# micropilot/myosuite-mjx

Hardware: AMD Instinct MI355X
Metric: env-steps/s (whole node) myoHandPoseRandom-v0 batch 4096 (higher is better)
Workload: dtype f32

## Files before the change

myosuite_mjx_amd/csrc/myo_hip.hip:

```cpp
#include "myo_common.h"
#include "myo_physics.h"
#include "myo_task_track.h"
#include "myo_kernel_lanes.h"
#include "myo_kernel_wave.h"
#include "myo_kernels_aux.h"
#include "myo_task_keyturn.h"
#include "myo_task_pen.h"
#include "myo_task_baoding.h"
#include "myo_task_myodm.h"

static int g_lanes = 64;
static thread_local std::string g_err;
static int fail(int code, const std::string& msg) { g_err = msg; return code; }
#define HIPCHK(x) do { hipError_t e_ = (x); if (e_ != hipSuccess) return fail(MYO_E_HIP, std::string(#x) + ": " + hipGetErrorString(e_)); } while (0)

struct BlobRec { char name[32]; uint32_t dtype, ndim, shape[4]; uint64_t nbytes, offset; };

struct myo_model {
  int device = 0;
  DevModel dm{};
  DevModelW dw{};
  DevModel* d_dm = nullptr;
  DevModelW* d_dw = nullptr;
  int env_lds_bytes_w = 0;
// ... 292 lines not shown
      for (size_t i = 0; i < dl.size() / 3; i++) {
        const int dd = dl[3 * i], sg = dl[3 * i + 1], slot = dl[3 * i + 2];
        if (dd < 0 || dd > 127 || slot < 0 || slot > 255 || sg < -32768 || sg > 32767) { myo_model_free(m); return fail(MYO_E_UNSUPPORTED, "moment-arm list entry does not fit the packed word"); }
        dlp[i] = dd | ((dof_type[dd] == 3 ? 1 : 0) << 7) | (slot << 8) | (int)((unsigned)sg << 16);
      }
      std::vector<int> dl4;
      std::vector<float> rec((size_t)std::max(d.nseg, 1) * SEGR * 4, 0.f);
      for (int idx = 0; idx < d.nseg; idx++) {
        const int si = seg_order[idx];
        const int* S = &seg[12 * (size_t)si];
        float* R = &rec[(size_t)idx * SEGR * 4];
        for (int k = 0; k < 2; k++) { R[4 * k] = fi(site_link[S[k]]); for (int c = 0; c < 3; c++) R[4 * k + 1 + c] = site_lpos[3 * (size_t)S[k] + c]; }
        R[8] = fi(S[2]); R[9] = fi(S[3] >= 0 ? site_link[S[3]] : -2); R[10] = 1.0f / seg_div[si]; R[11] = fi(seg_tendon[si]);
        for (int k = 0; k < 3; k++) {
          const int a0 = S[4 + 2 * k], n = S[5 + 2 * k], adr4 = (int)(dl4.size() / 4);
          if (adr4 >= (1 << 20) || n < 0 || n >= (1 << 11) || (n > 0 && (a0 < 0 || (size_t)(a0 + n) > dl.size() / 3))) { myo_model_free(m); return fail(MYO_E_UNSUPPORTED, "tendon moment-arm lists too long for the packed segment record"); }
          for (int i = 0; i < n; i++) dl4.push_back(dlp[a0 + i]);
          while (dl4.size() % 4 || dl4.size() == (size_t)adr4 * 4) dl4.push_back(0);
          R[12 + k] = fi(adr4 | (n << 20));
        }
        R[15] = fi(S[10]);
        if (S[2] >= 0) {
          const int g = S[2];
          if (S[3] >= 0) for (int c = 0; c < 3; c++) R[16 + c] = site_lpos[3 * (size_t)S[3] + c];
          R[19] = wg_radius[g];
          R[20] = fi(wg_link[g]); for (int c = 0; c < 3; c++) R[21 + c] = wg_lpos[3 * (size_t)g + c];
          for (int c = 0; c < 9; c++) R[24 + c] = wg_lmat[9 * (size_t)g + c];
        }
      }
      const float* tf4 = nullptr; const int* ti4 = nullptr;
      if (dl4.empty()) dl4.resize(4, 0);
      if ((rc = upload<float>(m, rec, &tf4)) || (rc = upload<int>(m, dl4, &ti4))) { myo_model_free(m); return rc; }
      w.seg_rec = (decltype(w.seg_rec))tf4; w.dl_pk = (decltype(w.dl_pk))ti4;
      const std::vector<int> cg_link = BI("hip_cg_link"), cg_type = BI("hip_cg_type"), pair_i = BI("hip_pair_i"), pair_dl = BI("hip_pair_dl");
      const std::vector<float> cg_lpos = BF("hip_cg_lpos"), cg_lmat = BF("hip_cg_lmat"), cg_size = BF("hip_cg_size"), cg_rb = BF("hip_cg_rbound"), pair_f = BF("hip_pair_f");
      std::vector<float> grec((size_t)std::max(d.ncg, 1) * 16, 0.f), prec((size_t)std::max(d.npair, 1) * 16, 0.f);
      for (int g = 0; g < d.ncg; g++) {
        float* R = &grec[(size_t)g * 16];
        R[0] = fi(cg_link[g]); for (int c = 0; c < 3; c++) R[1 + c] = cg_lpos[3 * (size_t)g + c];
        for (int c = 0; c < 9; c++) R[4 + c] = cg_lmat[9 * (size_t)g + c];
        R[13] = fi(cg_type[g]); R[14] = cg_rb[g];
      }
      for (int q = 0; q < d.npair; q++) {
        const int* P = &pair_i[6 * (size_t)q];
        const float* F = &pair_f[12 * (size_t)q];
        if (P[0] > 255 || P[1] > 255 || P[3] > 255 || P[4] > 15 || P[5] > 15) { myo_model_free(m); return fail(MYO_E_UNSUPPORTED, "collision pair does not fit the packed pair record"); }
        float* R = &prec[(size_t)q * 16];
        R[0] = fi(P[0] | (P[1] << 8) | (P[4] << 16) | (P[5] << 20) | (P[3] << 24)); R[1] = F[0]; R[2] = F[1]; R[3] = fi(P[2]);
        for (int c = 0; c < 3; c++) { R[4 + c] = cg_size[3 * (size_t)P[0] + c]; R[8 + c] = cg_size[3 * (size_t)P[1] + c]; }
        R[7] = cg_rb[P[0]]; R[11] = cg_rb[P[1]];
        R[12] = fi(cg_type[P[0]] | (cg_type[P[1]] << 8));
      }
      if (d.npair > 2048 || pair_dl.size() / 2 >= (1u << 16) || d.maxkc > 31) { myo_model_free(m); return fail(MYO_E_UNSUPPORTED, "more than 2048 collision pairs, 65535 contact dof-list entries or 31 dofs per contact"); }
      std::vector<int> pdl(std::max<size_t>(pair_dl.size() / 2, 1), 0);
      for (size_t i = 0; i < pair_dl.size() / 2; i++) {
        const int dd = pair_dl[2 * i], sg = pair_dl[2 * i + 1];
        if (dd < 0 || dd > 127 || sg < -(1 << 22) || sg > (1 << 22)) { myo_model_free(m); return fail(MYO_E_UNSUPPORTED, "contact dof-list entry does not fit the packed word"); }
        pdl[i] = dd | ((dof_type[dd] == 3 ? 1 : 0) << 7) | (int)((unsigned)sg << 8);
      }
      const float *tg4 = nullptr, *tp4 = nullptr; const int* tq4 = nullptr;
      if ((rc = upload<float>(m, grec, &tg4)) || (rc = upload<float>(m, prec, &tp4)) || (rc = upload<int>(m, pdl, &tq4))) { myo_model_free(m); return rc; }
      w.cg_rec = (decltype(w.cg_rec))tg4; w.pair_rec = (decltype(w.pair_rec))tp4; w.pair_dl_pk = (decltype(w.pair_dl_pk))tq4;
      {
        const std::vector<int> lpar = BI("hip_link_parent"), dlink = BI("hip_dof_link"), dpar = BI("dof_parentid"), kadr = BI("hip_kin_adr"), kvec = BI("hip_kin_vec"),
                               chadr = BI("hip_link_chain_adr"), chain = BI("hip_link_chain");
        if (d.nl > 64 || d.nv > 64) { myo_model_free(m); return fail(MYO_E_UNSUPPORTED, "more than 64 links or dofs"); }
// ... 1173 lines not shown
```

myosuite_mjx_amd/csrc/myo_kernel_wave.h:

```cpp
#ifndef MYO_KERNEL_WAVE_H
#define MYO_KERNEL_WAVE_H

#define NCONW 32
#define MPRW 14
static_assert(4 * MPRW <= 63, "the scheduler carries the table in a 64-word row (word 63 = entry count)");
struct LayW {
  int qpos, qvel, act, ctrl, lpos, lmat, axis, anchor, xv, qfc, sq, mprw, X;
  int tJ, tlen, tforce;
  int cdof, cinert, crb, cvel, cacc, cfrc;
  int gpos, gax, cand, cdist, cpos, cnrm, cpair, cJ, cdofs;
  int Mp;
  int tJp;
  int total;
};
__host__ __device__ constexpr LayW layout_w(int nq, int nv, int nu, int nl, int ngt, int maxnnz, int ncg, bool has_tl, int nvt, int kc, int nc, int nj) {
  LayW Y{};
  int o = 0;
  Y.qpos = o; o += nq; Y.qvel = o; o += nv; Y.act = o; o += nu; Y.ctrl = o; o += nu;
  Y.lpos = o; o += 3 * nl; Y.lmat = o; o += 9 * nl; Y.axis = o; o += 3 * nv; Y.anchor = o; o += 3 * nv;
  Y.xv = o; o += nvt; Y.qfc = o; o += nvt; Y.sq = o; o += nvt * (nvt + 1); Y.mprw = o; o += 4 * MPRW;
  Y.tJp = 0;
  if (has_tl) { Y.tJp = o; o += ngt * maxnnz + 2 * ngt; }
  Y.X = o;
  Y.tJ = o; o += ngt * maxnnz; Y.tlen = o; o += ngt; Y.tforce = o; o += nu;
// ... 11 lines not shown
  if (o < endT) o = endT;
  if (o < endD) o = endD;
  Y.total = o;
  return Y;
}
struct HfDev { int on, nrow, ncol, cg; float size[4], pos[3]; };
struct DevModelW {
  LayW lay;
  gpi seg_order, seg_tendon, gt_dl;
  gpf link_mat0;
  int nwrapseg, ndl, has_tl;
  gpf tl;
  int nq, has_free, neq;
  int has_j0;
  gpf gt_j0;
  HfDev hf;
  gpi link_free, dof_qposadr, eq_i, link_chain_adr, link_chain;
  int kin_dnmax;
  gpi kin_base, kin_adr, kin_vec;
  gpf eq_f;
  gpf mesh_rec, mesh_startrec, mesh_aabb;
  gpf fl, mesh_vert;
  gpf4 seg_rec;
  gpi dl_pk;
  gpf4 cg_rec;
  gpf4 pair_rec;
  gpi pair_dl_pk;
  gpi kin_pk;
  int kin_nround;
  gpi link_desc;
  gpi link_adof;
  gpi dof_anc;
  unsigned int free_rot[2], free_j3[2];
};
#define SEGR 9
#ifndef MPR_TOL
#define MPR_TOL 1e-8f
#endif

__device__ __forceinline__ float rdlane(float v, int l) { return __int_as_float(__builtin_amdgcn_readlane(__float_as_int(v), l)); }
__device__ __forceinline__ int rdlanei(int v, int l) { return __builtin_amdgcn_readlane(v, l); }
__device__ __forceinline__ float uniformf(float v) { return __int_as_float(__builtin_amdgcn_readfirstlane(__float_as_int(v))); }
template <int CTRL> __device__ __forceinline__ float dpp_add(float v) {
  return v + __int_as_float(__builtin_amdgcn_update_dpp(0, __float_as_int(v), CTRL, 0xf, 0xf, true));
}
__device__ __forceinline__ float wave_sum(float v) {
  v = dpp_add<0xB1>(v);
  v = dpp_add<0x4E>(v);
  v = dpp_add<0x141>(v);
  v = dpp_add<0x140>(v);
  return (rdlane(v, 0) + rdlane(v, 16)) + (rdlane(v, 32) + rdlane(v, 48));
}
#define WFOR(i, n) for (int i = lane; i < (n); i += 64)
__device__ __forceinline__ int wave_lane() {
  int l;
  asm volatile("v_mbcnt_lo_u32_b32 %0, -1, 0\n\tv_mbcnt_hi_u32_b32 %0, -1, %0" : "=v"(l));
  return l;
}
#define CDOF(E_, Y_, c_, k_) ((int)((((const unsigned int*)((E_) + (Y_).cdofs))[CDW * (c_) + ((k_) >> 2)] >> (8 * ((k_) & 3))) & 255u))
#define CDOFP(W_, k_) ((int)(((W_)[(k_) >> 2] >> (8 * ((k_) & 3))) & 255u))

template <int NVT> __device__ __forceinline__ float chol_rows(float (&r)[NVT], int lane) {
  float invd = 1.0f;
#pragma unroll
  for (int j = 0; j < NVT; j++) {
    const float pj = fmaxf(rdlane(r[j], j), MINVALF);
// ... 274 lines not shown
  const DevModel& M = *Mp;
  const DevModelW& W = *Wp;
  const LayC<SPEC, NVT, KC, NC, (TRK ? 4 : 3)> Yc{};
  const auto& Y = [&]() -> const auto& { if constexpr (SPEC != 0) return Yc; else return W.lay; }();
#define lane_id wave_lane()
  const int oe = (!SCHED && order) ? order[blockIdx.x] : blockIdx.x;
  int env = oe & 0x0FFFFFFF;
  if (!SCHED) {
    switch (oe >> 28) {
      case 3: __builtin_amdgcn_s_setprio(3); break;
      case 2: __builtin_amdgcn_s_setprio(2); break;
      case 1: __builtin_amdgcn_s_setprio(1); break;
      default: break;
    }
  }
  typedef Sizes<SPEC> Z;
  const int nv = SPEC ? Z::nv : M.nv, nu = SPEC ? Z::nu : M.nu, nq = SPEC ? Z::nq : W.nq;
  const int nl_ = SPEC ? Z::nl : M.nl, nlevel_ = SPEC ? Z::nlevel : M.nlevel, maxnnz_ = SPEC ? Z::maxnnz : M.maxnnz, ngt_ = SPEC ? Z::nu : M.ngt,
            nseg_ = SPEC ? Z::nseg : M.nseg, ncg_ = SPEC ? Z::ncg : M.ncg, npair_ = SPEC ? Z::npair : M.npair;
  constexpr int CDW = (KC + 3) / 4;
  constexpr int NJ = TRK ? 4 : 3;
  constexpr int NR = TRK ? 6 : 4;
  constexpr bool FULL = NVT > 24;
  const bool has_free = FULL && W.has_free;
  const int neq = FULL ? W.neq : 0;
  const bool has_tl = (SPEC != 0 || TRK) ? false : (W.has_tl != 0);
  const bool walk = FULL && wk != nullptr;
  if (!SCHED && FULL && (kflags & KF_RESET_ONLY) && Bt.elapsed[env] != 0) return;
#if MYO_STAMPS
  long long st_acc[12] = {0, 0, 0, 0, 0, 0, 0, 0, 0, 0, 0, 0};
  long long st_t0 = clock64();
  long long st_sub[12] = {0, 0, 0, 0, 0, 0, 0, 0, 0, 0, 0, 0}, st_s0 = 0;
  long long st_x[12] = {0, 0, 0, 0, 0, 0, 0, 0, 0, 0, 0, 0};
#define SUB0() do { st_s0 = clock64(); } while (0)
#define SUB(k) do { long long t1_ = clock64(); st_sub[k] += t1_ - st_s0; st_s0 = t1_; } while (0)
#define SUBX(k) do { long long t1_ = clock64(); st_x[k] += t1_ - st_s0; st_s0 = t1_; } while (0)
#define CNTX(k) do { st_x[k]++; } while (0)
#else
#define SUB0() do { } while (0)
#define SUB(k) do { } while (0)
#define SUBX(k) do { } while (0)
#define CNTX(k) do { } while (0)
#endif
  const int nsubtot = nsub + (walk ? 1 : 0);
  const float h = M.timestep;
  const int sq_q = SCHED ? (int)(__builtin_amdgcn_s_getreg((31 << 11) | 20) & 7) % S.nqueue : 0;
  int* const sq_ctl = SCHED ? S.ctl + 4 * sq_q : nullptr;
  int* const sq_ring = SCHED ? S.ring + (size_t)sq_q * S.stride : nullptr;
  const int sq_n = SCHED ? sq_ctl[2] : 0;
  int last_cost = 0;
  for (;;) {
  int s0 = 0, s1 = nsubtot;
  if (SCHED) {
    int t = 0;
    if (lane_id == 0) t = atomicAdd(&sq_ctl[0], 1);
    t = __builtin_amdgcn_readfirstlane(t);
    if (t >= sq_n * nsubtot) break;
    const int gen = t / sq_n, slot = t - gen * sq_n;
    int v = 0, spins = 0;
    for (;;) {
      v = __hip_atomic_load(&sq_ring[slot], __ATOMIC_RELAXED, __HIP_MEMORY_SCOPE_AGENT);
      if ((v >> 24) == gen || ++spins > (1 << 21)) break;
      __builtin_amdgcn_s_sleep(8);
    }
    v = __builtin_amdgcn_readfirstlane(v);
    if ((v >> 24) != gen) { if (lane_id == 0) { atomicOr(&Bt.flags[0], MYO_FLAG_SCHED_TIMEOUT); sq_ctl[3] = 1; } break; }
    env = v & SCHED_ENV_MASK;
    s0 = (v >> 20) & 15; s1 = s0 + 1;
  }
  float actdot[NTR];
  float* const warm_row = Bt.warm + (size_t)env * nv;
#pragma unroll
  for (int r = 0; r < NTR; r++) actdot[r] = 0.f;
#ifndef MYO_POISON_BITS
#define MYO_POISON_BITS 0x7fc00000
// ... 169 lines not shown
        }
        if (kind == 0) { E[Y.lmat + 9 * l + ix] = w[0]; E[Y.lmat + 9 * l + 3 + ix] = w[1]; E[Y.lmat + 9 * l + 6 + ix] = w[2]; }
        else {
          float* const dst = kind == 1 ? E + Y.lpos + 3 * l : (kind == 2 ? E + Y.axis + 3 * ix : E + Y.anchor + 3 * ix);
          dst[0] = w[0]; dst[1] = w[1]; dst[2] = w[2];
        }
      }
      SYNC();
    }
    if constexpr (TRK) {
      if (Bt.linkx && step == nsub - 1) {
        float* o = Bt.linkx + (size_t)env * 12 * nl_;
        for (int i = lane; i < 12 * nl_; i += 64) { const int l = i / 12, k = i - 12 * l; o[i] = k < 3 ? E[Y.lpos + 3 * l + k] + M.origin[k] : E[Y.lmat + 9 * l + (k - 3)]; }
      }
    }
    const float c0[3] = {has_free ? E[Y.lpos] : M.c0[0], has_free ? E[Y.lpos + 1] : M.c0[1], has_free ? E[Y.lpos + 2] : M.c0[2]};
    STAMP(1);
    SUB0();
    float tlen_r[NTR], tvel_r[NTR];
    if (W.has_j0) {
      WFOR(i, ngt_ * maxnnz_) E[Y.tJ + i] = W.gt_j0[i];
      WFOR(i, ngt_) {
        float L = M.gt_len0[i];
        for (int k = 0; k < maxnnz_; k++) { const float a = W.gt_j0[i * maxnnz_ + k]; if (a != 0.f) L += a * E[Y.qpos + W.dof_qposadr[M.gt_dofs[i * maxnnz_ + k]]]; }
        E[Y.tlen + i] = L;
      }
    } else {
    WFOR(i, ngt_ * maxnnz_) E[Y.tJ + i] = 0.f;
    WFOR(i, ngt_) E[Y.tlen + i] = M.gt_len0[i];
    }
    SYNC();
    for (int base = 0; base < nseg_; base += 64) {
      int idx = base + lane;
      if (idx < nseg_) {
        const gpf4 SR = W.seg_rec + (size_t)idx * SEGR;
        const float4 r0 = SR[0], r1 = SR[1], r2 = SR[2], r3 = SR[3];
        float4 r4 = r0, r5 = r0, r6 = r0, r7 = r0, r8 = r0;
        if (base < W.nwrapseg) { r4 = SR[4]; r5 = SR[5]; r6 = SR[6]; r7 = SR[7]; r8 = SR[8]; }
        const int g = __float_as_int(r2.x), side_l = __float_as_int(r2.y), gts = __float_as_int(r2.w);
        const float invdiv = r2.z;
        float p0[3], p1[3];
        { const float lp[3] = {r0.y, r0.z, r0.w}; frame_point(Y, E, __float_as_int(r0.x), lp, p0); }
        { const float lp[3] = {r1.y, r1.z, r1.w}; frame_point(Y, E, __float_as_int(r1.x), lp, p1); }
        const int wa = __float_as_int(r3.x), wb = __float_as_int(r3.y), wc = __float_as_int(r3.z);
        const gpi4 DL = (gpi4)W.dl_pk;
        const int4 ea = DL[wa & 0xFFFFF];
        int4 eb = ea, ec = ea;
        if (g >= 0) { eb = DL[wb & 0xFFFFF]; ec = DL[wc & 0xFFFFF]; }
        float wlen = -1, wp[6];
        if (g >= 0) {
          const int gl = __float_as_int(r5.x);
          const float glp[3] = {r5.y, r5.z, r5.w}, glm[9] = {r6.x, r6.y, r6.z, r6.w, r7.x, r7.y, r7.z, r7.w, r8.x};
          float gpos[3], gmat[9], side[3] = {0, 0, 0};
          if (gl < 0) {
#pragma unroll
            for (int k = 0; k < 3; k++) gpos[k] = glp[k];
#pragma unroll
            for (int k = 0; k < 9; k++) gmat[k] = glm[k];
          } else {
            float v[3];
            matvec(v, E + Y.lmat + 9 * gl, glp);
#pragma unroll
            for (int k = 0; k < 3; k++) gpos[k] = E[Y.lpos + 3 * gl + k] + v[k];
            matmul3(gmat, E + Y.lmat + 9 * gl, glm);
          }
          if (side_l != -2) { const float lp[3] = {r4.x, r4.y, r4.z}; frame_point(Y, E, side_l, lp, side); }
          wlen = wrap_geom_inl(wp, p0, p1, gpos, gmat, r4.w, __float_as_int(r3.w) != 0, side, side_l != -2);
        }
        SUB(7);
        bool wr = wlen >= 0;
        float* Jt = E + Y.tJ + gts * maxnnz_;
        float L = straight_w(W, Y, E, Jt, p0, p1, wa & 0xFFFFF, wa >> 20, invdiv, !wr, ea);
        if (g >= 0) {
          L += straight_w(W, Y, E, Jt, p0, wp, wb & 0xFFFFF, wb >> 20, invdiv, wr, eb);
          L += straight_w(W, Y, E, Jt, wp + 3, p1, wc & 0xFFFFF, wc >> 20, invdiv, wr, ec);
          if (wr) L += wlen * invdiv;
        }
        atomicAdd(&E[Y.tlen + gts], L);
      }
    }
    if (lane < nv) E[Y.qfc + lane] = 0.f;
    SYNC();
    SUB(8);
#pragma unroll
    for (int rr = 0; rr < NTR; rr++) {
      int gt = lane + 64 * rr;
      tlen_r[rr] = 0.f; tvel_r[rr] = 0.f;
      if (gt >= ngt_) continue;
      const float* Jrow = E + Y.tJ + gt * maxnnz_;
      const float L = E[Y.tlen + gt];
      tlen_r[rr] = L;
      float vel = 0;
      for (int k = 0; k < maxnnz_; k++) {
        int d = M.gt_dofs[gt * maxnnz_ + k];
        if (d >= 0) vel += Jrow[k] * E[Y.qvel + d];
        if (has_tl) E[Y.tJp + gt * maxnnz_ + k] = Jrow[k];
      }
      tvel_r[rr] = vel;
      if (has_tl) { E[Y.tJp + ngt_ * maxnnz_ + gt] = L; E[Y.tJp + ngt_ * maxnnz_ + ngt_ + gt] = vel; }
      if (gt < nu) {
        const float* A = M.act + 16 * gt;
        float f, ad;
        if (A[10] < 0.f) { f = A[0] * clipf(E[Y.ctrl + gt], A[12], A[13]) + A[1] + A[14] * (A[2] * L + A[3] * vel); ad = 0.f; }
        else muscle(A, A[14] * L, A[14] * vel, E[Y.act + gt], E[Y.ctrl + gt], &f, &ad);
        if constexpr (RK4) actdot[rr] = ad;
        else if (!op) E[Y.act + gt] += h * ad;
        const float ft = f * A[14];
        E[Y.tforce + gt] = ft;
        for (int k = 0; k < maxnnz_; k++) {
          const int d = M.gt_dofs[gt * maxnnz_ + k];
          if (d >= 0) atomicAdd(&E[Y.qfc + d], Jrow[k] * ft);
        }
      }
    }
    SYNC();
    const float qfa = lane < nv ? E[Y.qfc + lane] : 0.f;
    if (step == nsub - 1) {
      for (int i = lane; i < nu; i += 64) { Bt.tenlen[(size_t)env * nu + i] = E[Y.tlen + i]; Bt.actforce[(size_t)env * nu + i] = E[Y.tforce + i]; }
    }
    if (FULL && op) {
      float* o = Bt.obs + (size_t)env * wk->obs_dim + (nq - 2 + nv + 16);
#pragma unroll
      for (int rr = 0; rr < NTR; rr++) {
        int gt = lane + 64 * rr;
        if (gt < nu) {
          float g = M.act[16 * gt + 14];
          o[gt] = g * tlen_r[rr];
          o[nu + gt] = clipf(g * tvel_r[rr], -100.f, 100.f);
          o[2 * nu + gt] = clipf(E[Y.tforce + gt] / (g != 0.f ? g : 1.f) * 1e-3f, -100.f, 100.f);
          o[3 * nu + gt] = E[Y.act + gt];
        }
      }
    }
    SYNC();
    SUB(9);
    STAMP(2);
    typedef unsigned long long ull;
    constexpr bool M64 = NVT > 32;
    auto ld_mask = [&](gpi tab, int i) -> ull { const unsigned int lo = (unsigned int)tab[2 * i], hi = M64 ? (unsigned int)tab[2 * i + 1] : 0u; return (ull)lo | ((ull)hi << 32); };
    constexpr int BKG = SPEC ? (16 * Z::nl + 63) / 64 : 4;
    const ull adof_m = lane < nl_ ? ld_mask(W.link_adof, lane) : 0ull, anc_m = lane < nv ? ld_mask(W.dof_anc, lane) : 0ull;
    ull desc_m[BKG];
#pragma unroll
// ... 1615 lines not shown
```

myosuite_mjx_amd/csrc/myo_physics.h:

```cpp
#ifndef MYO_PHYSICS_H
#define MYO_PHYSICS_H

__device__ __forceinline__ bool is_intersect(const float* p1, const float* p2, const float* p3, const float* p4) {
  float det = (p4[1] - p3[1]) * (p2[0] - p1[0]) - (p4[0] - p3[0]) * (p2[1] - p1[1]);
  if (fabsf(det) < MINVALF) return false;
  float a = ((p4[0] - p3[0]) * (p1[1] - p3[1]) - (p4[1] - p3[1]) * (p1[0] - p3[0])) / det;
  float b = ((p2[0] - p1[0]) * (p1[1] - p3[1]) - (p2[1] - p1[1]) * (p1[0] - p3[0])) / det;
  return a >= 0 && a <= 1 && b >= 0 && b <= 1;
}

__device__ float wrap_circle(float* pnt, const float* d, const float* sd, bool has_side, float rad) {
  float sq0 = d[0] * d[0] + d[1] * d[1], sq1 = d[2] * d[2] + d[3] * d[3], sqr = rad * rad;
  if (sq0 < sqr || sq1 < sqr || rad < MINVALF) return -1;
  float dif[2] = {d[2] - d[0], d[3] - d[1]};
  float dd = dif[0] * dif[0] + dif[1] * dif[1];
  if (dd < MINVALF) return -1;
  float a = clipf(-(dif[0] * d[0] + dif[1] * d[1]) / dd, 0.f, 1.f);
  float tmp[2] = {a * dif[0] + d[0], a * dif[1] + d[1]};
  if (tmp[0] * tmp[0] + tmp[1] * tmp[1] > sqr && (!has_side || sd[0] * tmp[0] + sd[1] * tmp[1] >= 0)) return -1;
  float s0 = sqrtf(sq0 - sqr), s1 = sqrtf(sq1 - sqr);
  float sol[2][4], good[2];
  bool crossing[2];
#pragma unroll
  for (int i = 0; i < 2; i++) {
    float sgn = i == 0 ? 1.f : -1.f;
    sol[i][0] = (d[0] * sqr + sgn * rad * d[1] * s0) / sq0;
    sol[i][1] = (d[1] * sqr - sgn * rad * d[0] * s0) / sq0;
    sol[i][2] = (d[2] * sqr - sgn * rad * d[3] * s1) / sq1;
    sol[i][3] = (d[3] * sqr + sgn * rad * d[2] * s1) / sq1;
    if (has_side) {
      float t0 = sol[i][0] + sol[i][2], t1 = sol[i][1] + sol[i][3];
      const float c0 = sol[i][0] - sol[i][2], c1 = sol[i][1] - sol[i][3];
      const float n2 = t0 * t0 + t1 * t1, c2 = c0 * c0 + c1 * c1;
      if (n2 >= c2) {
        const float n = sqrtf(n2);
        if (n > MINVALF) { t0 /= n; t1 /= n; }
        good[i] = t0 * sd[0] + t1 * sd[1];
      } else {
        const float inv = __builtin_amdgcn_rsqf(c2), sg = (t1 * c0 - t0 * c1) < 0.f ? -1.f : 1.f;
        good[i] = sg * (c0 * sd[1] - c1 * sd[0]) * inv;
      }
    } else {
      float t0 = sol[i][0] - sol[i][2], t1 = sol[i][1] - sol[i][3];
      good[i] = -(t0 * t0 + t1 * t1);
    }
    float gz0 = sol[i][0] - sol[i][2], gz1 = sol[i][1] - sol[i][3];
    bool grazing = gz0 * gz0 + gz1 * gz1 < 1e-6f * sqr;
    crossing[i] = !grazing && is_intersect(d, sol[i], d + 2, sol[i] + 2);
    if (crossing[i]) good[i] = -10000.f;
  }
  int i = good[0] > good[1] ? 0 : 1;
#pragma unroll
  for (int k = 0; k < 4; k++) pnt[k] = i == 0 ? sol[0][k] : sol[1][k];
  if (i == 0 ? crossing[0] : crossing[1]) return -1;
  return rad * acosf(clipf((pnt[0] * pnt[2] + pnt[1] * pnt[3]) / sqr, -1.f, 1.f));
}

#ifndef MYO_EXACT_TRIG
#define MYO_EXACT_TRIG 0
#endif
__device__ __forceinline__ float asin01f(float x) {
  if (MYO_EXACT_TRIG) return asinf(fminf(x, 1.f));
  float p = -0.0012624911f;
  p = p * x + 0.0066700901f; p = p * x - 0.0170881256f; p = p * x + 0.0308918810f; p = p * x - 0.0501743046f;
  p = p * x + 0.0889789874f; p = p * x - 0.2145988016f; p = p * x + 1.5707963050f;
  return 1.57079632679f - sqrtf(fmaxf(0.f, 1.f - x)) * p;
}
__device__ __forceinline__ float acos11f(float x) {
  const float a = asin01f(fabsf(x));
  return x >= 0.f ? 1.57079632679f - a : 1.57079632679f + a;
}
__device__ __forceinline__ void sincos_q1f(float th, float* sn, float* cs) {
  if (MYO_EXACT_TRIG) { sincosf(th, sn, cs); return; }
  const bool hi = th > 0.785398163f;
  const float r = hi ? 1.57079632679f - th : th, z = r * r;
  const float s = r + r * z * (-1.6666654611e-1f + z * (8.3321608736e-3f + z * -1.9515295891e-4f));
  const float c = 1.f + z * (-0.5f + z * (4.166664568298827e-2f + z * (-1.388731625493765e-3f + z * 2.443315711809948e-5f)));
  *sn = hi ? c : s; *cs = hi ? s : c;
}
__device__ __forceinline__ void sincos_jf(float x, float* sn, float* cs) {
#ifdef MYO_KIN_LIBM
  sincosf(x, sn, cs); return;
#endif
  if (MYO_EXACT_TRIG) { sincosf(x, sn, cs); return; }
  const float k = rintf(x * 0.636619772367581343f);
  float r = fmaf(-k, 1.57079637050628662109375f, x);
  r = fmaf(-k, -4.37113882867379116e-8f, r);
  const float z = r * r;
  const float s = r + r * z * (-1.6666654611e-1f + z * (8.3321608736e-3f + z * -1.9515295891e-4f));
  const float c = 1.f + z * (-0.5f + z * (4.166664568298827e-2f + z * (-1.388731625493765e-3f + z * 2.443315711809948e-5f)));
  const int q = (int)k;
  const float a = (q & 1) ? c : s, b = (q & 1) ? s : c;
  *sn = (q & 2) ? -a : a;
  *cs = ((q + 1) & 2) ? -b : b;
}
__device__ float wrap_inside(float* pnt, const float* d, float rad) {
  const float zinit = 1.f - 1e-7f, tolerance = 1e-6f;
  float len0 = sqrtf(d[0] * d[0] + d[1] * d[1]), len1 = sqrtf(d[2] * d[2] + d[3] * d[3]);
  float dif[2] = {d[2] - d[0], d[3] - d[1]};
  float dd = dif[0] * dif[0] + dif[1] * dif[1];
  if (len0 <= rad || len1 <= rad || rad < MINVALF || len0 < MINVALF || len1 < MINVALF) return -1;
  if (dd > MINVALF) {
    float a = -(dif[0] * d[0] + dif[1] * d[1]) / dd;
    if (a > 0 && a < 1) {
      float t0 = a * dif[0] + d[0], t1 = a * dif[1] + d[1];
      if (sqrtf(t0 * t0 + t1 * t1) <= rad) return -1;
    }
  }
  pnt[0] = 0.5f * (d[0] + d[2]); pnt[1] = 0.5f * (d[1] + d[3]);
  float n = sqrtf(pnt[0] * pnt[0] + pnt[1] * pnt[1]);
  if (n > MINVALF) { pnt[0] *= rad / n; pnt[1] *= rad / n; }
  pnt[2] = pnt[0]; pnt[3] = pnt[1];
  float A = rad / len0, B = rad / len1;
  float cosG = (len0 * len0 + len1 * len1 - dd) / (2 * len0 * len1);
  if (cosG < -1 + MINVALF) return -1;
  if (cosG > 1 - MINVALF) return 0;
  float Gang = acos11f(cosG);
  (void)zinit;
  float th = 1.57079632679f - 4.4721360e-4f;
  float sn = 0.9999999f, cs = 4.4721359e-4f;
  float f = asin01f(A * sn) + asin01f(B * sn) - 2 * th + Gang;
  if (f > 0) return 0;
  for (int iter = 0; iter < 20 && fabsf(f) > tolerance; iter++) {
    float df = A * cs / fmaxf(MINVALF, sqrtf(1 - A * A * sn * sn)) + B * cs / fmaxf(MINVALF, sqrtf(1 - B * B * sn * sn)) - 2;
    th = clipf(th - f / df, 1e-6f, 1.57079632679f);
    sincos_q1f(th, &sn, &cs);
    f = asin01f(A * sn) + asin01f(B * sn) - 2 * th + Gang;
  }
  float vec[2], ang;
  if (d[0] * d[3] - d[1] * d[2] > 0) { vec[0] = d[0] / len0; vec[1] = d[1] / len0; ang = th - asin01f(A * sn); }
  else { vec[0] = d[2] / len1; vec[1] = d[3] / len1; ang = th - asin01f(B * sn); }
  float sa, ca;
  sincos_q1f(clipf(ang, 0.f, 1.57079632679f), &sa, &ca);
  pnt[0] = rad * (ca * vec[0] - sa * vec[1]);
  pnt[1] = rad * (sa * vec[0] + ca * vec[1]);
  pnt[2] = pnt[0]; pnt[3] = pnt[1];
  return 0;
}

#define MYO_WRAP_GEOM_BODY  \
  float p[6], s[3] = {0, 0, 0}, tmp[3], axis[6], d[4], sd[2] = {0, 0}, pnt[4], res[6];  \
  tmp[0] = x0[0] - xpos[0]; tmp[1] = x0[1] - xpos[1]; tmp[2] = x0[2] - xpos[2];  \
  matTvec(p, xmat, tmp);  \
  tmp[0] = x1[0] - xpos[0]; tmp[1] = x1[1] - xpos[1]; tmp[2] = x1[2] - xpos[2];  \
  matTvec(p + 3, xmat, tmp);  \
  if (norm3(p) < MINVALF || norm3(p + 3) < MINVALF) return -1;  \
  if (has_side) {  \
    tmp[0] = side[0] - xpos[0]; tmp[1] = side[1] - xpos[1]; tmp[2] = side[2] - xpos[2];  \
    matTvec(s, xmat, tmp);  \
  }  \
  if (!cylinder) {  \
    axis[0] = p[0]; axis[1] = p[1]; axis[2] = p[2];  \
    normalize3(axis);  \
    float nrmv[3];  \
    cross3(nrmv, p, p + 3);  \
    float nrm = norm3(nrmv);  \
    if (nrm < MINVALF) {  \
      int i = 0;  \
      if (fabsf(axis[1]) > fabsf(axis[0]) && fabsf(axis[1]) > fabsf(axis[2])) i = 1;  \
      if (fabsf(axis[2]) > fabsf(axis[0]) && fabsf(axis[2]) > fabsf(axis[1])) i = 2;  \
      float t[3] = {i == 0 ? 0.f : 1.f, i == 1 ? 0.f : 1.f, i == 2 ? 0.f : 1.f};  \
      cross3(nrmv, axis, t);  \
      nrm = norm3(nrmv);  \
    }  \
    float inv = 1.0f / nrm;  \
    nrmv[0] *= inv; nrmv[1] *= inv; nrmv[2] *= inv;  \
    cross3(axis + 3, nrmv, axis);    \
    d[0] = dot3(p, axis); d[1] = dot3(p, axis + 3); d[2] = dot3(p + 3, axis); d[3] = dot3(p + 3, axis + 3);  \
    if (has_side) { sd[0] = dot3(s, axis); sd[1] = dot3(s, axis + 3); }  \
  } else {  \
    d[0] = p[0]; d[1] = p[1]; d[2] = p[3]; d[3] = p[4];  \
    if (has_side) { sd[0] = s[0]; sd[1] = s[1]; }  \
  }  \
  float wlen;  \
  float sdn = sqrtf(sd[0] * sd[0] + sd[1] * sd[1]);  \
  if (has_side && sdn < radius) {  \
    wlen = wrap_inside(pnt, d, radius);  \
  } else {  \
    if (has_side && sdn > MINVALF) { sd[0] /= sdn; sd[1] /= sdn; }  \
    wlen = wrap_circle(pnt, d, sd, has_side, radius);  \
  }  \
  if (wlen < 0) return -1;  \
  if (!cylinder) {  \
_Pragma("unroll")  \
    for (int k = 0; k < 3; k++) {  \
      res[k] = axis[k] * pnt[0] + axis[3 + k] * pnt[1];  \
      res[3 + k] = axis[k] * pnt[2] + axis[3 + k] * pnt[3];  \
    }  \
  } else {  \
    float L0 = sqrtf((p[0] - pnt[0]) * (p[0] - pnt[0]) + (p[1] - pnt[1]) * (p[1] - pnt[1]));  \
    float L1 = sqrtf((p[3] - pnt[2]) * (p[3] - pnt[2]) + (p[4] - pnt[3]) * (p[4] - pnt[3]));  \
    float tot = L0 + wlen + L1;  \
    res[0] = pnt[0]; res[1] = pnt[1]; res[3] = pnt[2]; res[4] = pnt[3];  \
    res[2] = p[2] + (p[5] - p[2]) * L0 / tot;  \
    res[5] = p[2] + (p[5] - p[2]) * (L0 + wlen) / tot;  \
    float h = res[5] - res[2];  \
    wlen = sqrtf(wlen * wlen + h * h);  \
  }  \
  matvec(wpnt, xmat, res);  \
  matvec(wpnt + 3, xmat, res + 3);  \
_Pragma("unroll")  \
  for (int k = 0; k < 3; k++) { wpnt[k] += xpos[k]; wpnt[3 + k] += xpos[k]; }  \
  return wlen;

__device__ float wrap_geom(float* wpnt, const float* x0, const float* x1, const float* xpos, const float* xmat, float radius,
                           bool cylinder, const float* side, bool has_side) {
  MYO_WRAP_GEOM_BODY
}
__device__ __forceinline__ float wrap_geom_inl(float* wpnt, const float* x0, const float* x1, const float* xpos, const float* xmat, float radius,
                                               bool cylinder, const float* side, bool has_side) {
  MYO_WRAP_GEOM_BODY
}

__device__ __forceinline__ float muscle_fl(float L, float lmin, float lmax) {
  if (lmin <= L && L <= lmax) {
    float a = 0.5f * (lmin + 1), b = 0.5f * (1 + lmax), x;
    if (L <= a) { x = (L - lmin) / fmaxf(MINVALF, a - lmin); return 0.5f * x * x; }
    else if (L <= 1) { x = (1 - L) / fmaxf(MINVALF, 1 - a); return 1 - 0.5f * x * x; }
    else if (L <= b) { x = (L - 1) / fmaxf(MINVALF, b - 1); return 1 - 0.5f * x * x; }
    else { x = (lmax - L) / fmaxf(MINVALF, lmax - b); return 0.5f * x * x; }
  }
  return 0;
}
__device__ __forceinline__ void muscle(const float* A, float len, float vel, float act, float ctrl, float* force, float* actdot) {
  float r0 = A[0], r1 = A[1], F0 = A[2], lmin = A[3], lmax = A[4], vmax = A[5], fpmax = A[6], fvmax = A[7], lr0 = A[8], lr1 = A[9];
  float L0 = (lr1 - lr0) / fmaxf(MINVALF, r1 - r0);
  float L = r0 + (len - lr0) / fmaxf(MINVALF, L0);
  float V = vel / fmaxf(MINVALF, L0 * vmax);
  float FL = muscle_fl(L, lmin, lmax), FV, y = fvmax - 1;
  if (V <= -1) FV = 0;
  else if (V <= 0) FV = (V + 1) * (V + 1);
  else if (V <= y) FV = fvmax - (y - V) * (y - V) / fmaxf(MINVALF, y);
  else FV = fvmax;
  float gain = -F0 * FL * FV;
  float b = 0.5f * (1 + lmax), bias, x;
  if (L <= 1) bias = 0;
  else if (L <= b) { x = (L - 1) / fmaxf(MINVALF, b - 1); bias = -A[15] * fpmax * 0.5f * x * x; }
  else { x = (L - b) / fmaxf(MINVALF, b - 1); bias = -A[15] * fpmax * (0.5f + x); }
  *force = gain * act + bias;
  float cc = clipf(clipf(ctrl, A[12], A[13]), 0.f, 1.f), ac = clipf(act, 0.f, 1.f);
  float tau_act = A[10] * (0.5f + 1.5f * ac), tau_deact = A[11] / (0.5f + 1.5f * ac);
  float dctrl = cc - act;
  *actdot = dctrl / fmaxf(MINVALF, dctrl > 0 ? tau_act : tau_deact);
}
// ... 454 lines not shown
```

Before: 4.462 million.

## Branch-free wrap-geom solve, byte-packed tendon dof lists, register-cached actuator params

Replaces the inlined wrap-geometry macro with a variant that computes both the sphere and cylinder frame paths unconditionally and selects results, and merges the inside and circle solver prologues into one shared computation. The aim is to cut lane divergence when segments of different wrap types share a wave. Tendon dof indices are packed into bytes and loaded as int4 records in the specialised path, and actuator parameters are loaded into registers with float4 loads. It also adds optional clock-stamp instrumentation for the wrap phases. The cost is redundant math on every lane and more register pressure.

```diff
diff --git a/myosuite_mjx_amd/csrc/myo_hip.hip b/myosuite_mjx_amd/csrc/myo_hip.hip
--- a/myosuite_mjx_amd/csrc/myo_hip.hip
+++ b/myosuite_mjx_amd/csrc/myo_hip.hip
@@ -348,6 +348,21 @@
       if (dl4.empty()) dl4.resize(4, 0);
       if ((rc = upload<float>(m, rec, &tf4)) || (rc = upload<int>(m, dl4, &ti4))) { myo_model_free(m); return rc; }
       w.seg_rec = (decltype(w.seg_rec))tf4; w.dl_pk = (decltype(w.dl_pk))ti4;
+      {
+        const std::vector<int> gt_dofs = BI("hip_gt_dofs");
+        const int rows = (d.maxnnz + 15) / 16;
+        std::vector<int> gdp((size_t)std::max(d.ngt, 1) * rows * 4, -1);
+        if (gt_dofs.size() < (size_t)d.ngt * d.maxnnz) { myo_model_free(m); return fail(MYO_E_BLOB, "model blob lacks hip_gt_dofs"); }
+        for (int t = 0; t < d.ngt; t++)
+          for (int k = 0; k < d.maxnnz; k++) {
+            const int v = gt_dofs[(size_t)t * d.maxnnz + k];
+            if (v < -1 || v > 127) { myo_model_free(m); return fail(MYO_E_UNSUPPORTED, "tendon dof list entry does not fit the packed byte"); }
+            ((unsigned char*)&gdp[(size_t)t * rows * 4])[k] = (unsigned char)(v < 0 ? 0xFF : v);
+          }
+        const int* tg = nullptr;
+        if ((rc = upload<int>(m, gdp, &tg))) { myo_model_free(m); return rc; }
+        w.gt_dof_pk = (decltype(w.gt_dof_pk))tg;
+      }
       const std::vector<int> cg_link = BI("hip_cg_link"), cg_type = BI("hip_cg_type"), pair_i = BI("hip_pair_i"), pair_dl = BI("hip_pair_dl");
       const std::vector<float> cg_lpos = BF("hip_cg_lpos"), cg_lmat = BF("hip_cg_lmat"), cg_size = BF("hip_cg_size"), cg_rb = BF("hip_cg_rbound"), pair_f = BF("hip_pair_f");
       std::vector<float> grec((size_t)std::max(d.ncg, 1) * 16, 0.f), prec((size_t)std::max(d.npair, 1) * 16, 0.f);
diff --git a/myosuite_mjx_amd/csrc/myo_kernel_wave.h b/myosuite_mjx_amd/csrc/myo_kernel_wave.h
--- a/myosuite_mjx_amd/csrc/myo_kernel_wave.h
+++ b/myosuite_mjx_amd/csrc/myo_kernel_wave.h
@@ -67,6 +67,7 @@
   gpi link_adof;
   gpi dof_anc;
   unsigned int free_rot[2], free_j3[2];
+  gpi gt_dof_pk;
 };
 #define SEGR 9
 #ifndef MPR_TOL
@@ -407,15 +408,20 @@
   long long st_t0 = clock64();
   long long st_sub[12] = {0, 0, 0, 0, 0, 0, 0, 0, 0, 0, 0, 0}, st_s0 = 0;
   long long st_x[12] = {0, 0, 0, 0, 0, 0, 0, 0, 0, 0, 0, 0};
+  long long st_w = 0;
 #define SUB0() do { st_s0 = clock64(); } while (0)
 #define SUB(k) do { long long t1_ = clock64(); st_sub[k] += t1_ - st_s0; st_s0 = t1_; } while (0)
 #define SUBX(k) do { long long t1_ = clock64(); st_x[k] += t1_ - st_s0; st_s0 = t1_; } while (0)
 #define CNTX(k) do { st_x[k]++; } while (0)
+#define WSUB0() do { st_w = clock64(); } while (0)
+#define WSUB(k) do { long long t1_ = clock64(); st_x[3 + (k)] += t1_ - st_w; st_w = t1_; } while (0)
 #else
 #define SUB0() do { } while (0)
 #define SUB(k) do { } while (0)
 #define SUBX(k) do { } while (0)
 #define CNTX(k) do { } while (0)
+#define WSUB0() do { } while (0)
+#define WSUB(k) do { } while (0)
 #endif
   const int nsubtot = nsub + (walk ? 1 : 0);
   const float h = M.timestep;
@@ -651,6 +657,7 @@
     SYNC();
     for (int base = 0; base < nseg_; base += 64) {
       int idx = base + lane;
+      WSUB0();
       if (idx < nseg_) {
         const gpf4 SR = W.seg_rec + (size_t)idx * SEGR;
         const float4 r0 = SR[0], r1 = SR[1], r2 = SR[2], r3 = SR[3];
@@ -684,7 +691,8 @@
             matmul3(gmat, E + Y.lmat + 9 * gl, glm);
           }
           if (side_l != -2) { const float lp[3] = {r4.x, r4.y, r4.z}; frame_point(Y, E, side_l, lp, side); }
-          wlen = wrap_geom_inl(wp, p0, p1, gpos, gmat, r4.w, __float_as_int(r3.w) != 0, side, side_l != -2);
+          WSUB(0);
+          wlen = wrap_geom_w(wp, p0, p1, gpos, gmat, r4.w, __float_as_int(r3.w) != 0, side, side_l != -2, [&](int k) { WSUB(1 + k); });
         }
         SUB(7);
         bool wr = wlen >= 0;
@@ -697,28 +705,51 @@
         }
         atomicAdd(&E[Y.tlen + gts], L);
       }
+      WSUB(3);
     }
     if (lane < nv) E[Y.qfc + lane] = 0.f;
     SYNC();
     SUB(8);
+    constexpr int GDR = SPEC ? (Z::maxnnz + 15) / 16 : 1;
 #pragma unroll
     for (int rr = 0; rr < NTR; rr++) {
       int gt = lane + 64 * rr;
       tlen_r[rr] = 0.f; tvel_r[rr] = 0.f;
       if (gt >= ngt_) continue;
+      int4 dr[GDR];
+      if constexpr (SPEC != 0) {
+#pragma unroll
+        for (int j = 0; j < GDR; j++) dr[j] = ((gpi4)W.gt_dof_pk)[GDR * gt + j];
+      }
+      const float* A = M.act + 16 * gt;
+      float Ar[16];
+      if constexpr (SPEC != 0) {
+        if (gt < nu) {
+          const gpf4 A4 = (gpf4)A;
+#pragma unroll
+          for (int j = 0; j < 4; j++) { const float4 a = A4[j]; Ar[4 * j] = a.x; Ar[4 * j + 1] = a.y; Ar[4 * j + 2] = a.z; Ar[4 * j + 3] = a.w; }
+        }
+        A = Ar;
+      }
+      auto gdof = [&](int k) -> int {
+        if constexpr (SPEC != 0) {
+          const int4 q = dr[k >> 4];
+          const int w = (k & 15) < 8 ? ((k & 15) < 4 ? q.x : q.y) : ((k & 15) < 12 ? q.z : q.w);
+          return (int)(signed char)(w >> (8 * (k & 3)));
+        } else return M.gt_dofs[gt * maxnnz_ + k];
+      };
       const float* Jrow = E + Y.tJ + gt * maxnnz_;
       const float L = E[Y.tlen + gt];
       tlen_r[rr] = L;
       float vel = 0;
       for (int k = 0; k < maxnnz_; k++) {
-        int d = M.gt_dofs[gt * maxnnz_ + k];
+        const int d = gdof(k);
         if (d >= 0) vel += Jrow[k] * E[Y.qvel + d];
         if (has_tl) E[Y.tJp + gt * maxnnz_ + k] = Jrow[k];
       }
       tvel_r[rr] = vel;
       if (has_tl) { E[Y.tJp + ngt_ * maxnnz_ + gt] = L; E[Y.tJp + ngt_ * maxnnz_ + ngt_ + gt] = vel; }
       if (gt < nu) {
-        const float* A = M.act + 16 * gt;
         float f, ad;
         if (A[10] < 0.f) { f = A[0] * clipf(E[Y.ctrl + gt], A[12], A[13]) + A[1] + A[14] * (A[2] * L + A[3] * vel); ad = 0.f; }
         else muscle(A, A[14] * L, A[14] * vel, E[Y.act + gt], E[Y.ctrl + gt], &f, &ad);
@@ -727,7 +758,7 @@
         const float ft = f * A[14];
         E[Y.tforce + gt] = ft;
         for (int k = 0; k < maxnnz_; k++) {
-          const int d = M.gt_dofs[gt * maxnnz_ + k];
+          const int d = gdof(k);
           if (d >= 0) atomicAdd(&E[Y.qfc + d], Jrow[k] * ft);
         }
       }
diff --git a/myosuite_mjx_amd/csrc/myo_physics.h b/myosuite_mjx_amd/csrc/myo_physics.h
--- a/myosuite_mjx_amd/csrc/myo_physics.h
+++ b/myosuite_mjx_amd/csrc/myo_physics.h
@@ -9,15 +9,7 @@
   return a >= 0 && a <= 1 && b >= 0 && b <= 1;
 }
 
-__device__ float wrap_circle(float* pnt, const float* d, const float* sd, bool has_side, float rad) {
-  float sq0 = d[0] * d[0] + d[1] * d[1], sq1 = d[2] * d[2] + d[3] * d[3], sqr = rad * rad;
-  if (sq0 < sqr || sq1 < sqr || rad < MINVALF) return -1;
-  float dif[2] = {d[2] - d[0], d[3] - d[1]};
-  float dd = dif[0] * dif[0] + dif[1] * dif[1];
-  if (dd < MINVALF) return -1;
-  float a = clipf(-(dif[0] * d[0] + dif[1] * d[1]) / dd, 0.f, 1.f);
-  float tmp[2] = {a * dif[0] + d[0], a * dif[1] + d[1]};
-  if (tmp[0] * tmp[0] + tmp[1] * tmp[1] > sqr && (!has_side || sd[0] * tmp[0] + sd[1] * tmp[1] >= 0)) return -1;
+__device__ __forceinline__ float wrap_circle_tail(float* pnt, const float* d, const float* sd, bool has_side, float rad, float sq0, float sq1, float sqr) {
   float s0 = sqrtf(sq0 - sqr), s1 = sqrtf(sq1 - sqr);
   float sol[2][4], good[2];
   bool crossing[2];
@@ -55,6 +47,17 @@
   if (i == 0 ? crossing[0] : crossing[1]) return -1;
   return rad * acosf(clipf((pnt[0] * pnt[2] + pnt[1] * pnt[3]) / sqr, -1.f, 1.f));
 }
+__device__ float wrap_circle(float* pnt, const float* d, const float* sd, bool has_side, float rad) {
+  float sq0 = d[0] * d[0] + d[1] * d[1], sq1 = d[2] * d[2] + d[3] * d[3], sqr = rad * rad;
+  if (sq0 < sqr || sq1 < sqr || rad < MINVALF) return -1;
+  float dif[2] = {d[2] - d[0], d[3] - d[1]};
+  float dd = dif[0] * dif[0] + dif[1] * dif[1];
+  if (dd < MINVALF) return -1;
+  float a = clipf(-(dif[0] * d[0] + dif[1] * d[1]) / dd, 0.f, 1.f);
+  float tmp[2] = {a * dif[0] + d[0], a * dif[1] + d[1]};
+  if (tmp[0] * tmp[0] + tmp[1] * tmp[1] > sqr && (!has_side || sd[0] * tmp[0] + sd[1] * tmp[1] >= 0)) return -1;
+  return wrap_circle_tail(pnt, d, sd, has_side, rad, sq0, sq1, sqr);
+}
 
 #ifndef MYO_EXACT_TRIG
 #define MYO_EXACT_TRIG 0
@@ -94,19 +97,8 @@
   *sn = (q & 2) ? -a : a;
   *cs = ((q + 1) & 2) ? -b : b;
 }
-__device__ float wrap_inside(float* pnt, const float* d, float rad) {
+__device__ __forceinline__ float wrap_inside_tail(float* pnt, const float* d, float rad, float len0, float len1, float dd) {
   const float zinit = 1.f - 1e-7f, tolerance = 1e-6f;
-  float len0 = sqrtf(d[0] * d[0] + d[1] * d[1]), len1 = sqrtf(d[2] * d[2] + d[3] * d[3]);
-  float dif[2] = {d[2] - d[0], d[3] - d[1]};
-  float dd = dif[0] * dif[0] + dif[1] * dif[1];
-  if (len0 <= rad || len1 <= rad || rad < MINVALF || len0 < MINVALF || len1 < MINVALF) return -1;
-  if (dd > MINVALF) {
-    float a = -(dif[0] * d[0] + dif[1] * d[1]) / dd;
-    if (a > 0 && a < 1) {
-      float t0 = a * dif[0] + d[0], t1 = a * dif[1] + d[1];
-      if (sqrtf(t0 * t0 + t1 * t1) <= rad) return -1;
-    }
-  }
   pnt[0] = 0.5f * (d[0] + d[2]); pnt[1] = 0.5f * (d[1] + d[3]);
   float n = sqrtf(pnt[0] * pnt[0] + pnt[1] * pnt[1]);
   if (n > MINVALF) { pnt[0] *= rad / n; pnt[1] *= rad / n; }
@@ -137,79 +129,161 @@
   pnt[2] = pnt[0]; pnt[3] = pnt[1];
   return 0;
 }
-
-#define MYO_WRAP_GEOM_BODY  \
-  float p[6], s[3] = {0, 0, 0}, tmp[3], axis[6], d[4], sd[2] = {0, 0}, pnt[4], res[6];  \
-  tmp[0] = x0[0] - xpos[0]; tmp[1] = x0[1] - xpos[1]; tmp[2] = x0[2] - xpos[2];  \
-  matTvec(p, xmat, tmp);  \
-  tmp[0] = x1[0] - xpos[0]; tmp[1] = x1[1] - xpos[1]; tmp[2] = x1[2] - xpos[2];  \
-  matTvec(p + 3, xmat, tmp);  \
-  if (norm3(p) < MINVALF || norm3(p + 3) < MINVALF) return -1;  \
-  if (has_side) {  \
-    tmp[0] = side[0] - xpos[0]; tmp[1] = side[1] - xpos[1]; tmp[2] = side[2] - xpos[2];  \
-    matTvec(s, xmat, tmp);  \
-  }  \
-  if (!cylinder) {  \
-    axis[0] = p[0]; axis[1] = p[1]; axis[2] = p[2];  \
-    normalize3(axis);  \
-    float nrmv[3];  \
-    cross3(nrmv, p, p + 3);  \
-    float nrm = norm3(nrmv);  \
-    if (nrm < MINVALF) {  \
-      int i = 0;  \
-      if (fabsf(axis[1]) > fabsf(axis[0]) && fabsf(axis[1]) > fabsf(axis[2])) i = 1;  \
-      if (fabsf(axis[2]) > fabsf(axis[0]) && fabsf(axis[2]) > fabsf(axis[1])) i = 2;  \
-      float t[3] = {i == 0 ? 0.f : 1.f, i == 1 ? 0.f : 1.f, i == 2 ? 0.f : 1.f};  \
-      cross3(nrmv, axis, t);  \
-      nrm = norm3(nrmv);  \
-    }  \
-    float inv = 1.0f / nrm;  \
-    nrmv[0] *= inv; nrmv[1] *= inv; nrmv[2] *= inv;  \
-    cross3(axis + 3, nrmv, axis);    \
-    d[0] = dot3(p, axis); d[1] = dot3(p, axis + 3); d[2] = dot3(p + 3, axis); d[3] = dot3(p + 3, axis + 3);  \
-    if (has_side) { sd[0] = dot3(s, axis); sd[1] = dot3(s, axis + 3); }  \
-  } else {  \
-    d[0] = p[0]; d[1] = p[1]; d[2] = p[3]; d[3] = p[4];  \
-    if (has_side) { sd[0] = s[0]; sd[1] = s[1]; }  \
-  }  \
-  float wlen;  \
-  float sdn = sqrtf(sd[0] * sd[0] + sd[1] * sd[1]);  \
-  if (has_side && sdn < radius) {  \
-    wlen = wrap_inside(pnt, d, radius);  \
-  } else {  \
-    if (has_side && sdn > MINVALF) { sd[0] /= sdn; sd[1] /= sdn; }  \
-    wlen = wrap_circle(pnt, d, sd, has_side, radius);  \
-  }  \
-  if (wlen < 0) return -1;  \
-  if (!cylinder) {  \
-_Pragma("unroll")  \
-    for (int k = 0; k < 3; k++) {  \
-      res[k] = axis[k] * pnt[0] + axis[3 + k] * pnt[1];  \
-      res[3 + k] = axis[k] * pnt[2] + axis[3 + k] * pnt[3];  \
-    }  \
-  } else {  \
-    float L0 = sqrtf((p[0] - pnt[0]) * (p[0] - pnt[0]) + (p[1] - pnt[1]) * (p[1] - pnt[1]));  \
-    float L1 = sqrtf((p[3] - pnt[2]) * (p[3] - pnt[2]) + (p[4] - pnt[3]) * (p[4] - pnt[3]));  \
-    float tot = L0 + wlen + L1;  \
-    res[0] = pnt[0]; res[1] = pnt[1]; res[3] = pnt[2]; res[4] = pnt[3];  \
-    res[2] = p[2] + (p[5] - p[2]) * L0 / tot;  \
-    res[5] = p[2] + (p[5] - p[2]) * (L0 + wlen) / tot;  \
-    float h = res[5] - res[2];  \
-    wlen = sqrtf(wlen * wlen + h * h);  \
-  }  \
-  matvec(wpnt, xmat, res);  \
-  matvec(wpnt + 3, xmat, res + 3);  \
-_Pragma("unroll")  \
-  for (int k = 0; k < 3; k++) { wpnt[k] += xpos[k]; wpnt[3 + k] += xpos[k]; }  \
-  return wlen;
+__device__ float wrap_inside(float* pnt, const float* d, float rad) {
+  float len0 = sqrtf(d[0] * d[0] + d[1] * d[1]), len1 = sqrtf(d[2] * d[2] + d[3] * d[3]);
+  float dif[2] = {d[2] - d[0], d[3] - d[1]};
+  float dd = dif[0] * dif[0] + dif[1] * dif[1];
+  if (len0 <= rad || len1 <= rad || rad < MINVALF || len0 < MINVALF || len1 < MINVALF) return -1;
+  if (dd > MINVALF) {
+    float a = -(dif[0] * d[0] + dif[1] * d[1]) / dd;
+    if (a > 0 && a < 1) {
+      float t0 = a * dif[0] + d[0], t1 = a * dif[1] + d[1];
+      if (sqrtf(t0 * t0 + t1 * t1) <= rad) return -1;
+    }
+  }
+  return wrap_inside_tail(pnt, d, rad, len0, len1, dd);
+}
+__device__ __forceinline__ float wrap_solve_w(float* pnt, const float* d, const float* sd, bool has_side, bool inside, float rad) {
+  const float sq0 = d[0] * d[0] + d[1] * d[1], sq1 = d[2] * d[2] + d[3] * d[3], sqr = rad * rad;
+  const float dif[2] = {d[2] - d[0], d[3] - d[1]};
+  const float dd = dif[0] * dif[0] + dif[1] * dif[1];
+  const float a = -(dif[0] * d[0] + dif[1] * d[1]) / dd, ac = clipf(a, 0.f, 1.f);
+  const float t0 = ac * dif[0] + d[0], t1 = ac * dif[1] + d[1], tn2 = t0 * t0 + t1 * t1;
+  if (inside) {
+    const float len0 = sqrtf(sq0), len1 = sqrtf(sq1);
+    if (len0 <= rad || len1 <= rad || rad < MINVALF || len0 < MINVALF || len1 < MINVALF) return -1;
+    if (dd > MINVALF && a > 0 && a < 1 && sqrtf(tn2) <= rad) return -1;
+    return wrap_inside_tail(pnt, d, rad, len0, len1, dd);
+  }
+  if (sq0 < sqr || sq1 < sqr || rad < MINVALF || dd < MINVALF) return -1;
+  if (tn2 > sqr && (!has_side || sd[0] * t0 + sd[1] * t1 >= 0)) return -1;
+  return wrap_circle_tail(pnt, d, sd, has_side, rad, sq0, sq1, sqr);
+}
 
 __device__ float wrap_geom(float* wpnt, const float* x0, const float* x1, const float* xpos, const float* xmat, float radius,
                            bool cylinder, const float* side, bool has_side) {
-  MYO_WRAP_GEOM_BODY
-}
-__device__ __forceinline__ float wrap_geom_inl(float* wpnt, const float* x0, const float* x1, const float* xpos, const float* xmat, float radius,
-                                               bool cylinder, const float* side, bool has_side) {
-  MYO_WRAP_GEOM_BODY
+  float p[6], s[3] = {0, 0, 0}, tmp[3], axis[6], d[4], sd[2] = {0, 0}, pnt[4], res[6];
+  tmp[0] = x0[0] - xpos[0]; tmp[1] = x0[1] - xpos[1]; tmp[2] = x0[2] - xpos[2];
+  matTvec(p, xmat, tmp);
+  tmp[0] = x1[0] - xpos[0]; tmp[1] = x1[1] - xpos[1]; tmp[2] = x1[2] - xpos[2];
+  matTvec(p + 3, xmat, tmp);
+  if (norm3(p) < MINVALF || norm3(p + 3) < MINVALF) return -1;
+  if (has_side) {
+    tmp[0] = side[0] - xpos[0]; tmp[1] = side[1] - xpos[1]; tmp[2] = side[2] - xpos[2];
+    matTvec(s, xmat, tmp);
+  }
+  if (!cylinder) {
+    axis[0] = p[0]; axis[1] = p[1]; axis[2] = p[2];
+    normalize3(axis);
+    float nrmv[3];
+    cross3(nrmv, p, p + 3);
+    float nrm = norm3(nrmv);
+    if (nrm < MINVALF) {
+      int i = 0;
+      if (fabsf(axis[1]) > fabsf(axis[0]) && fabsf(axis[1]) > fabsf(axis[2])) i = 1;
+      if (fabsf(axis[2]) > fabsf(axis[0]) && fabsf(axis[2]) > fabsf(axis[1])) i = 2;
+      float t[3] = {i == 0 ? 0.f : 1.f, i == 1 ? 0.f : 1.f, i == 2 ? 0.f : 1.f};
+      cross3(nrmv, axis, t);
+      nrm = norm3(nrmv);
+    }
+    float inv = 1.0f / nrm;
+    nrmv[0] *= inv; nrmv[1] *= inv; nrmv[2] *= inv;
+    cross3(axis + 3, nrmv, axis);
+    d[0] = dot3(p, axis); d[1] = dot3(p, axis + 3); d[2] = dot3(p + 3, axis); d[3] = dot3(p + 3, axis + 3);
+    if (has_side) { sd[0] = dot3(s, axis); sd[1] = dot3(s, axis + 3); }
+  } else {
+    d[0] = p[0]; d[1] = p[1]; d[2] = p[3]; d[3] = p[4];
+    if (has_side) { sd[0] = s[0]; sd[1] = s[1]; }
+  }
+  float wlen;
+  float sdn = sqrtf(sd[0] * sd[0] + sd[1] * sd[1]);
+  if (has_side && sdn < radius) {
+    wlen = wrap_inside(pnt, d, radius);
+  } else {
+    if (has_side && sdn > MINVALF) { sd[0] /= sdn; sd[1] /= sdn; }
+    wlen = wrap_circle(pnt, d, sd, has_side, radius);
+  }
+  if (wlen < 0) return -1;
+  if (!cylinder) {
+#pragma unroll
+    for (int k = 0; k < 3; k++) {
+      res[k] = axis[k] * pnt[0] + axis[3 + k] * pnt[1];
+      res[3 + k] = axis[k] * pnt[2] + axis[3 + k] * pnt[3];
+    }
+  } else {
+    float L0 = sqrtf((p[0] - pnt[0]) * (p[0] - pnt[0]) + (p[1] - pnt[1]) * (p[1] - pnt[1]));
+    float L1 = sqrtf((p[3] - pnt[2]) * (p[3] - pnt[2]) + (p[4] - pnt[3]) * (p[4] - pnt[3]));
+    float tot = L0 + wlen + L1;
+    res[0] = pnt[0]; res[1] = pnt[1]; res[3] = pnt[2]; res[4] = pnt[3];
+    res[2] = p[2] + (p[5] - p[2]) * L0 / tot;
+    res[5] = p[2] + (p[5] - p[2]) * (L0 + wlen) / tot;
+    float h = res[5] - res[2];
+    wlen = sqrtf(wlen * wlen + h * h);
+  }
+  matvec(wpnt, xmat, res);
+  matvec(wpnt + 3, xmat, res + 3);
+#pragma unroll
+  for (int k = 0; k < 3; k++) { wpnt[k] += xpos[k]; wpnt[3 + k] += xpos[k]; }
+  return wlen;
+}
+template <class MK>
+__device__ __forceinline__ float wrap_geom_w(float* wpnt, const float* x0, const float* x1, const float* xpos, const float* xmat, float radius,
+                                             bool cylinder, const float* side, bool has_side, MK&& mark) {
+  float p[6], s[3] = {0, 0, 0}, tmp[3], axis[6], d[4], sd[2] = {0, 0}, pnt[4], res[6];
+  tmp[0] = x0[0] - xpos[0]; tmp[1] = x0[1] - xpos[1]; tmp[2] = x0[2] - xpos[2];
+  matTvec(p, xmat, tmp);
+  tmp[0] = x1[0] - xpos[0]; tmp[1] = x1[1] - xpos[1]; tmp[2] = x1[2] - xpos[2];
+  matTvec(p + 3, xmat, tmp);
+  if (norm3(p) < MINVALF || norm3(p + 3) < MINVALF) return -1;
+  if (has_side) {
+    tmp[0] = side[0] - xpos[0]; tmp[1] = side[1] - xpos[1]; tmp[2] = side[2] - xpos[2];
+    matTvec(s, xmat, tmp);
+  }
+  axis[0] = p[0]; axis[1] = p[1]; axis[2] = p[2];
+  normalize3(axis);
+  float nrmv[3];
+  cross3(nrmv, p, p + 3);
+  float nrm = norm3(nrmv);
+  if (!cylinder && nrm < MINVALF) {
+    int i = 0;
+    if (fabsf(axis[1]) > fabsf(axis[0]) && fabsf(axis[1]) > fabsf(axis[2])) i = 1;
+    if (fabsf(axis[2]) > fabsf(axis[0]) && fabsf(axis[2]) > fabsf(axis[1])) i = 2;
+    float t[3] = {i == 0 ? 0.f : 1.f, i == 1 ? 0.f : 1.f, i == 2 ? 0.f : 1.f};
+    cross3(nrmv, axis, t);
+    nrm = norm3(nrmv);
+  }
+  float inv = 1.0f / nrm;
+  nrmv[0] *= inv; nrmv[1] *= inv; nrmv[2] *= inv;
+  cross3(axis + 3, nrmv, axis);
+  if (cylinder) { axis[0] = 1.f; axis[1] = 0.f; axis[2] = 0.f; axis[3] = 0.f; axis[4] = 1.f; axis[5] = 0.f; }
+  d[0] = dot3(p, axis); d[1] = dot3(p, axis + 3); d[2] = dot3(p + 3, axis); d[3] = dot3(p + 3, axis + 3);
+  if (has_side) { sd[0] = dot3(s, axis); sd[1] = dot3(s, axis + 3); }
+  mark(0);
+  float sdn = sqrtf(sd[0] * sd[0] + sd[1] * sd[1]);
+  const bool inside = has_side && sdn < radius;
+  if (!inside && has_side && sdn > MINVALF) { sd[0] /= sdn; sd[1] /= sdn; }
+  float wlen = wrap_solve_w(pnt, d, sd, has_side, inside, radius);
+  mark(1);
+  if (wlen < 0) return -1;
+#pragma unroll
+  for (int k = 0; k < 3; k++) {
+    res[k] = axis[k] * pnt[0] + axis[3 + k] * pnt[1];
+    res[3 + k] = axis[k] * pnt[2] + axis[3 + k] * pnt[3];
+  }
+  {
+    float L0 = sqrtf((p[0] - pnt[0]) * (p[0] - pnt[0]) + (p[1] - pnt[1]) * (p[1] - pnt[1]));
+    float L1 = sqrtf((p[3] - pnt[2]) * (p[3] - pnt[2]) + (p[4] - pnt[3]) * (p[4] - pnt[3]));
+    float tot = L0 + wlen + L1;
+    const float z0 = p[2] + (p[5] - p[2]) * L0 / tot, z1 = p[2] + (p[5] - p[2]) * (L0 + wlen) / tot;
+    float h = z1 - z0;
+    const float wc = sqrtf(wlen * wlen + h * h);
+    if (cylinder) { res[2] = z0; res[5] = z1; wlen = wc; }
+  }
+  matvec(wpnt, xmat, res);
+  matvec(wpnt + 3, xmat, res + 3);
+#pragma unroll
+  for (int k = 0; k < 3; k++) { wpnt[k] += xpos[k]; wpnt[3 + k] += xpos[k]; }
+  return wlen;
 }
 
 __device__ __forceinline__ float muscle_fl(float L, float lmin, float lmax) {
```

Result: no change. 4.466 million, median of 3 (+0.1%).
